# Orbis-Tertius/tiny-ram-halo2

Measured on AMD Instinct MI355X. Metric: Pallas MSM pairs/s @ 2^24 + Fp NTT elems/s @ 2^22; 1/2/4/8 MI355X, higher is better.
Workload: dtype u255 (255-bit modular integers as 9 x 29/30-bit limbs in i32 / i64 lanes)

## Files before the change

tiny-ram-halo2_amd/csrc/msm.hip:

```cpp
#include <stdlib.h>
#include <string.h>

#include "ctx.h"
#include "devmem.h"
#include "curve_q4.h"
#include "hostcombine.h"
#include "hosthelper.h"
#include "hostplan.h"

namespace trh {

namespace {

using hostplan::MAX_C; using hostplan::MAX_C_FIXED; using hostplan::MSM_TILE; using hostplan::SMALL_C; using hostplan::SMALL_MAX_N;
using hostplan::PART_TILE; using hostplan::BIN_THREADS; using hostplan::BIN_PER_MAX; using hostplan::BIN_CAP_MAX; using hostplan::RANGE_BLOCK;
using hostplan::HEAVY_PIECES; using hostplan::SP_LISTS; using hostplan::SP_CNT; using hostplan::SP_PAD; using hostplan::SP_PARTS; using hostplan::SP_MAX_CHUNK;
using hostplan::num_windows;
static_assert(sizeof(XYZZMem) == hostplan::XYZZ_BYTES && sizeof(XYZZzMem) == hostplan::RAW_POINT_BYTES, "point sizes of the plan's scratch layout");
constexpr u32 SIGN_BIT = 0x80000000u;

template <class SF>
__global__ void __launch_bounds__(256) msm_recode_kernel(const uint4* __restrict__ scalars, size_t n, int mont, int c, int W,
                                                         u32* __restrict__ digits, u32* __restrict__ bin_counts, int k2, u32 nbins, int use_lds, size_t sstride,
                                                         int one_row ,
                                                         const uint4* __restrict__ tails ,
                                                         unsigned char* __restrict__ tile_flags ,
                                                         u32 tile_log, u32 tiles) {
    const size_t z = blockIdx.z;
    const u32 rows = one_row ? 1u : (u32)W;
    scalars += z * sstride * 2; digits += z * (size_t)W * n; bin_counts += z * (size_t)rows * nbins;
    extern __shared__ u32 lhist[];
    const u32 total = rows * nbins;
    if (use_lds) {
        for (u32 k = threadIdx.x; k < total; k += blockDim.x) lhist[k] = 0;
        __syncthreads();
    }
    const u32 mask = (1u << c) - 1u, half = 1u << (c - 1);
    for (size_t i = (size_t)blockIdx.x * blockDim.x + threadIdx.x; i < n; i += (size_t)gridDim.x * blockDim.x) {
        const uint4* src = (tails && i == n - 1) ? tails + 2 * z : scalars + 2 * i;
        uint4 lo = src[0], hi = src[1];
        u32 w[8] = {lo.x, lo.y, lo.z, lo.w, hi.x, hi.y, hi.z, hi.w};
        if (mont) fe_store(fe_from_mont(fe_load<SF>(w)), w);
        u32 carry = 0;
        for (int j = 0; j < W; ++j) {
            u32 raw = (w[0] & mask) + carry;
#pragma unroll
            for (int k = 0; k < 7; ++k) w[k] = (w[k] >> c) | (w[k + 1] << (32 - c));
            w[7] >>= c;
            u32 bucket, sign = 0;
            if (raw > half) { bucket = (1u << c) - raw; carry = 1; sign = SIGN_BIT; }
            else { bucket = raw; carry = 0; }
            digits[(size_t)j * n + i] = bucket ? (bucket | sign) : 0u;
            if (tile_flags) {
                const unsigned long long nz = __ballot(bucket != 0);
                const size_t slot = (size_t)j * n + i;
                const u32 lane = threadIdx.x & 63u;
                if (bucket && ((nz & ((1ull << lane) - 1ull)) == 0ull || (slot & (((size_t)1 << tile_log) - 1)) < 64))
                    tile_flags[z * tiles + (slot >> tile_log)] = 1;
            }
            if (bucket) {
                const u32 bin = (bucket - 1u) >> k2, row = one_row ? 0u : (u32)j;
                if (use_lds) atomicAdd(&lhist[row * nbins + bin], 1u);
                else atomicAdd(&bin_counts[(size_t)row * nbins + bin], 1u);
            }
        }
    }
    if (use_lds) {
        __syncthreads();
        for (u32 k = threadIdx.x; k < total; k += blockDim.x) {
            const u32 v = lhist[k];
            if (v) atomicAdd(&bin_counts[k], v);
        }
    }
}

struct ZeroRanges { uint4* p[4]; u32 n16[4]; };
__global__ void __launch_bounds__(256) msm_zero_ranges_kernel(const ZeroRanges z) {
    const uint4 zero = make_uint4(0, 0, 0, 0);
#pragma unroll
    for (int k = 0; k < 4; ++k)
        for (u32 i = blockIdx.x * blockDim.x + threadIdx.x; i < z.n16[k]; i += gridDim.x * blockDim.x) z.p[k][i] = zero;
}

__global__ void __launch_bounds__(1024) msm_offsets_kernel(u32* __restrict__ counts, u32* __restrict__ starts, u32 nb1, u32* __restrict__ oversize, u32 bin_cap,
                                                           u32* __restrict__ totals ) {
    const size_t z = blockIdx.z;
    counts += z * (size_t)gridDim.x * nb1; starts += z * (size_t)gridDim.x * nb1;
    __shared__ u32 part[1024];
    const int j = blockIdx.x, t = threadIdx.x;
    u32* cnt = counts + (size_t)j * nb1;
    u32* st = starts + (size_t)j * nb1;
    const u32 per = (nb1 + 1023u) / 1024u;
    const u32 lo = t * per < nb1 ? t * per : nb1, hi = (lo + per < nb1) ? lo + per : nb1;
    u32 sum = 0, biggest = 0;
    for (u32 b = lo; b < hi; ++b) { const u32 v = cnt[b]; sum += v; biggest = v > biggest ? v : biggest; }
    if (oversize && biggest > bin_cap) atomicMax(oversize + z * gridDim.x + blockIdx.x, biggest);
    part[t] = sum;
    __syncthreads();
    for (int off = 1; off < 1024; off <<= 1) {
        u32 v = (t >= off) ? part[t - off] : 0;
        __syncthreads();
        part[t] += v;
        __syncthreads();
    }
    if (totals && t == 1023) totals[z * gridDim.x + blockIdx.x] = part[1023];
    u32 run = part[t] - sum;
    for (u32 b = lo; b < hi; ++b) {
        u32 cv = cnt[b];
        st[b] = run;
        cnt[b] = run;
        run += cv;
    }
}

constexpr int PART_THREADS = 1024;
__global__ void __launch_bounds__(PART_THREADS) msm_partition_kernel(const u32* __restrict__ digits, u32* __restrict__ bin_cursor,
                                                                     u32* __restrict__ parted, size_t n, int k2, u32 nbins, int idx_bits,
                                                                     const unsigned char* __restrict__ tile_flags ) {
    const size_t z = blockIdx.z;
    if (tile_flags && !tile_flags[z * gridDim.x + blockIdx.x]) return;
    digits += z * (size_t)gridDim.y * n; parted += z * (size_t)gridDim.y * n; bin_cursor += z * (size_t)gridDim.y * nbins;
    extern __shared__ u32 lds[];
    u32* stage = lds;
    u32* cnt = lds + PART_TILE;
    u32* lbase = cnt + nbins;
    u32* gbase = lbase + nbins;
    __shared__ u32 scan[PART_THREADS];
    const int j = blockIdx.y;
    const size_t t0 = (size_t)blockIdx.x * PART_TILE;
    const size_t t1 = t0 + PART_TILE < n ? t0 + PART_TILE : n;
    const u32* dg = digits + (size_t)j * n;
    for (u32 k = threadIdx.x; k < nbins; k += blockDim.x) cnt[k] = 0;
    __syncthreads();
    constexpr int PER = PART_TILE / PART_THREADS;
    u32 mine[PER];
#pragma unroll
    for (int q = 0; q < PER; ++q) {
        const size_t i = t0 + threadIdx.x + (size_t)q * PART_THREADS;
        mine[q] = i < t1 ? dg[i] : 0u;
    }
#pragma unroll
    for (int q = 0; q < PER; ++q) {
        const u32 b = mine[q] & ~SIGN_BIT;
        if (b) atomicAdd(&cnt[(b - 1u) >> k2], 1u);
    }
    __syncthreads();
    {
        const u32 per = (nbins + PART_THREADS - 1) / PART_THREADS;
        const u32 lo = threadIdx.x * per < nbins ? threadIdx.x * per : nbins, hi = lo + per < nbins ? lo + per : nbins;
        u32 sum = 0;
        for (u32 k = lo; k < hi; ++k) sum += cnt[k];
        scan[threadIdx.x] = sum;
        __syncthreads();
        for (int off = 1; off < PART_THREADS; off <<= 1) {
            const u32 v = ((int)threadIdx.x >= off) ? scan[threadIdx.x - off] : 0;
            __syncthreads();
            scan[threadIdx.x] += v;
            __syncthreads();
        }
        u32 run = scan[threadIdx.x] - sum;
        for (u32 k = lo; k < hi; ++k) {
            const u32 v = cnt[k];
            lbase[k] = run;
            gbase[k] = v ? atomicAdd(&bin_cursor[(size_t)j * nbins + k], v) : 0u;
            run += v;
        }
    }
    __syncthreads();
    for (u32 k = threadIdx.x; k < nbins; k += blockDim.x) cnt[k] = 0;
    __syncthreads();
    const u32 low_mask = (1u << k2) - 1u;
#pragma unroll
    for (int q = 0; q < PER; ++q) {
        const u32 e = mine[q];
        const u32 b = e & ~SIGN_BIT;
        if (b) {
            const u32 bm = b - 1u, bin = bm >> k2;
            const u32 r = atomicAdd(&cnt[bin], 1u);
            stage[lbase[bin] + r] = (u32)(t0 + threadIdx.x + (size_t)q * PART_THREADS) | ((bm & low_mask) << idx_bits) | (e & SIGN_BIT);
        }
    }
    __syncthreads();
    u32* out = parted + (size_t)j * n;
    const u32 wave = threadIdx.x >> 6, lane = threadIdx.x & 63u;
    for (u32 bin = wave; bin < nbins; bin += PART_THREADS / 64) {
        const u32 c = cnt[bin], lb = lbase[bin], gb = gbase[bin];
        for (u32 k = lane; k < c; k += 64) out[gb + k] = stage[lb + k];
    }
}

constexpr int BS_CHUNK = 8192;
constexpr int BS_THREADS = 512;

__device__ __forceinline__ u32 bin_of_position(const u32* __restrict__ bin_ends, u32 nbins, u32 pos) {
    u32 lo = 0, hi = nbins;
    while (lo < hi) {
        const u32 mid = (lo + hi) >> 1;
        if (bin_ends[mid] > pos) hi = mid; else lo = mid + 1;
    }
    return lo;
}

template <bool SCATTER>
__global__ void __launch_bounds__(BS_THREADS) msm_bucket_pass_kernel(const u32* __restrict__ parted, const u32* __restrict__ bin_starts,
                                                                     const u32* __restrict__ bin_ends, u32* __restrict__ bucket_cnt ,
                                                                     u32* __restrict__ sorted, size_t n, int k2, u32 nbins, int idx_bits, u32 nbk,
                                                                     const u32* __restrict__ oversize) {
    const size_t z = blockIdx.z;
    {
        const size_t Wz = gridDim.y;
        parted += z * Wz * n; sorted += z * Wz * n; bin_starts += z * Wz * nbins; bin_ends += z * Wz * nbins;
        bucket_cnt += z * Wz * (nbk + 1);
    }
    if (oversize && oversize[z * gridDim.y + blockIdx.y] == 0u) return;
    __shared__ u32 cnt[128], tbase[128], gbase[128];
    __shared__ u32 stage[SCATTER ? BS_CHUNK : 1];
    const int j = blockIdx.y;
    const u32* bs = bin_starts + (size_t)j * nbins;
    const u32* be = bin_ends + (size_t)j * nbins;
    const u32 total = be[nbins - 1];
    const u32 c0 = blockIdx.x * BS_CHUNK;
    if (c0 >= total) return;
    const u32 c1 = c0 + BS_CHUNK < total ? c0 + BS_CHUNK : total;
    const u32 nsub = 1u << k2, low_mask = nsub - 1u, idx_mask = (1u << idx_bits) - 1u;
    const u32* src = parted + (size_t)j * n;
    u32* dst = sorted + (size_t)j * n;
    u32* bc = bucket_cnt + (size_t)j * (nbk + 1);
    const u32 wave = threadIdx.x >> 6, lane = threadIdx.x & 63u;
    for (u32 bin = bin_of_position(be, nbins, c0); bin < nbins; ++bin) {
        const u32 lo = bs[bin] > c0 ? bs[bin] : c0;
        if (lo >= c1) break;
        const u32 hi = be[bin] < c1 ? be[bin] : c1;
        if (hi <= lo) continue;
        if (hi - lo <= 64u) {
            if (threadIdx.x < hi - lo) {
                const u32 e = src[lo + threadIdx.x];
                u32* cell = &bc[(bin << k2) + ((e >> idx_bits) & low_mask) + 1u];
                if (!SCATTER) atomicAdd(cell, 1u);
                else dst[atomicAdd(cell, 1u)] = (e & idx_mask) | (e & SIGN_BIT);
            }
            continue;
        }
        if (threadIdx.x < 128) cnt[threadIdx.x] = 0;
        __syncthreads();
        for (u32 i = lo + threadIdx.x; i < hi; i += blockDim.x) atomicAdd(&cnt[(src[i] >> idx_bits) & low_mask], 1u);
        __syncthreads();
        if (!SCATTER) {
            if (threadIdx.x < nsub && cnt[threadIdx.x]) atomicAdd(&bc[(bin << k2) + threadIdx.x + 1u], cnt[threadIdx.x]);
        } else {
            if (threadIdx.x == 0) {
                u32 r = 0;
                for (u32 k = 0; k < nsub; ++k) { tbase[k] = r; r += cnt[k]; }
            }
            if (threadIdx.x < nsub) {
                const u32 v = cnt[threadIdx.x];
                gbase[threadIdx.x] = v ? atomicAdd(&bc[(bin << k2) + threadIdx.x + 1u], v) : 0u;
            }
            __syncthreads();
            if (threadIdx.x < 128) cnt[threadIdx.x] = 0;
            __syncthreads();
            for (u32 i = lo + threadIdx.x; i < hi; i += blockDim.x) {
                const u32 e = src[i];
                const u32 sub = (e >> idx_bits) & low_mask;
                const u32 r = atomicAdd(&cnt[sub], 1u);
                stage[tbase[sub] + r] = (e & idx_mask) | (e & SIGN_BIT);
            }
            __syncthreads();
            for (u32 sub = wave; sub < nsub; sub += BS_THREADS / 64) {
                const u32 c = cnt[sub], sb = tbase[sub], gb = gbase[sub];
                for (u32 k = lane; k < c; k += 64) dst[gb + k] = stage[sb + k];
            }
        }
        __syncthreads();
    }
}

template <int PER>
__global__ void __launch_bounds__(BIN_THREADS) msm_bin_sort_kernel(const u32* __restrict__ parted, const u32* __restrict__ bin_starts, const u32* __restrict__ bin_ends,
                                                                   u32* __restrict__ sorted, u32* __restrict__ starts, u32* __restrict__ ends, size_t n, int k2, u32 nbins,
                                                                   int idx_bits, u32 nbk, const u32* __restrict__ oversize) {
    if (oversize[(size_t)blockIdx.z * gridDim.y + blockIdx.y] != 0u) return;
    extern __shared__ u32 bstage[];
    __shared__ u32 cnt[128], tbase[128], wave0_total;
    const size_t z = blockIdx.z, Wz = gridDim.y;
    const int j = blockIdx.y;
    const u32 bin = blockIdx.x;
    const size_t wrow = z * Wz + j;
    const u32 lo = bin_starts[wrow * nbins + bin], hi = bin_ends[wrow * nbins + bin];
    const u32 count = hi - lo;
    const u32 nsub = 1u << k2, low_mask = nsub - 1u, idx_mask = (1u << idx_bits) - 1u;
    const u32* src = parted + wrow * n + lo;
    u32* dst = sorted + wrow * n + lo;
    const u32 lane = threadIdx.x & 63u;
    if (threadIdx.x < 128) cnt[threadIdx.x] = 0;
    __syncthreads();
    u32 mine[PER];
#pragma unroll
    for (int q = 0; q < PER; ++q) {
        const u32 i = threadIdx.x + (u32)q * BIN_THREADS;
        mine[q] = (u32)q * BIN_THREADS < count ? src[i < count ? i : 0u] : 0u;
    }
#pragma unroll
    for (int q = 0; q < PER; ++q)
        if (threadIdx.x + (u32)q * BIN_THREADS < count) atomicAdd(&cnt[(mine[q] >> idx_bits) & low_mask], 1u);
    __syncthreads();
    u32 v = 0, x = 0;
    if (threadIdx.x < 128) {
        v = threadIdx.x < nsub ? cnt[threadIdx.x] : 0u;
        x = v;
#pragma unroll
        for (int off = 1; off < 64; off <<= 1) {
            const u32 y = __shfl_up(x, off, 64);
            if ((int)lane >= off) x += y;
        }
        if (threadIdx.x == 63) wave0_total = x;
    }
    __syncthreads();
    if (threadIdx.x < 128) {
        const u32 excl = x - v + (threadIdx.x >= 64 ? wave0_total : 0u);
        tbase[threadIdx.x] = excl;
        cnt[threadIdx.x] = 0;
        if (threadIdx.x < nsub) {
            const size_t b = wrow * (nbk + 1) + ((size_t)bin << k2) + threadIdx.x + 1u;
            starts[b] = lo + excl;
            ends[b] = lo + excl + v;
        }
        if (bin == 0 && threadIdx.x == 0) { starts[wrow * (nbk + 1)] = 0; ends[wrow * (nbk + 1)] = 0; }
    }
    __syncthreads();
#pragma unroll
    for (int q = 0; q < PER; ++q) {
        if (threadIdx.x + (u32)q * BIN_THREADS < count) {
            const u32 e = mine[q];
            const u32 sub = (e >> idx_bits) & low_mask;
            const u32 r = atomicAdd(&cnt[sub], 1u);
            bstage[tbase[sub] + r] = (e & idx_mask) | (e & SIGN_BIT);
        }
    }
    __syncthreads();
#pragma unroll
    for (int q = 0; q < PER; ++q) {
        const u32 i = threadIdx.x + (u32)q * BIN_THREADS;
        if (i < count) mine[q] = bstage[i];
    }
#pragma unroll
    for (int q = 0; q < PER; ++q) {
        const u32 i = threadIdx.x + (u32)q * BIN_THREADS;
        if (i < count) dst[i] = mine[q];
    }
}

__global__ void __launch_bounds__(RANGE_BLOCK) msm_bucket_block_sums_kernel(const u32* __restrict__ bucket_cnt, u32* __restrict__ block_sums, u32 nbk,
                                                                            const u32* __restrict__ oversize) {
    if (oversize && oversize[(size_t)blockIdx.z * gridDim.y + blockIdx.y] == 0u) return;
    __shared__ u32 part[RANGE_BLOCK / 64];
    const size_t z = blockIdx.z, Wz = gridDim.y;
    const u32 nb1 = nbk + 1, b = blockIdx.x * RANGE_BLOCK + threadIdx.x;
    u32 v = b < nb1 ? bucket_cnt[(z * Wz + blockIdx.y) * nb1 + b] : 0u;
#pragma unroll
    for (int off = 32; off > 0; off >>= 1) v += __shfl_down(v, off, 64);
    if ((threadIdx.x & 63) == 0) part[threadIdx.x >> 6] = v;
    __syncthreads();
    if (threadIdx.x == 0) {
        u32 t = 0;
        for (int k = 0; k < RANGE_BLOCK / 64; ++k) t += part[k];
        block_sums[(z * Wz + blockIdx.y) * gridDim.x + blockIdx.x] = t;
    }
}
__global__ void __launch_bounds__(RANGE_BLOCK) msm_bucket_ranges_kernel(u32* __restrict__ bucket_cnt, const u32* __restrict__ block_sums, u32* __restrict__ starts,
                                                                        u32* __restrict__ ends, u32 nbk, const u32* __restrict__ oversize) {
    if (oversize && oversize[(size_t)blockIdx.z * gridDim.y + blockIdx.y] == 0u) return;
    __shared__ u32 part[RANGE_BLOCK];
    __shared__ u32 before;
    const size_t z = blockIdx.z, Wz = gridDim.y;
    const int t = threadIdx.x;
    const u32 nb1 = nbk + 1, b = blockIdx.x * RANGE_BLOCK + t;
    const size_t row = (z * Wz + blockIdx.y) * nb1;
    const u32 c = b < nb1 ? bucket_cnt[row + b] : 0u;
    {
        u32 v = (u32)t < blockIdx.x ? block_sums[(z * Wz + blockIdx.y) * gridDim.x + t] : 0u;
        part[t] = v;
        __syncthreads();
        for (int s = RANGE_BLOCK / 2; s > 0; s >>= 1) {
            if (t < s) part[t] += part[t + s];
            __syncthreads();
        }
        if (t == 0) before = part[0];
        __syncthreads();
    }
    part[t] = c;
    __syncthreads();
    for (int off = 1; off < RANGE_BLOCK; off <<= 1) {
        const u32 v = (t >= off) ? part[t - off] : 0;
        __syncthreads();
        part[t] += v;
        __syncthreads();
    }
    if (b < nb1) {
        const u32 E = before + part[t], S = E - c;
        starts[row + b] = S; ends[row + b] = E; bucket_cnt[row + b] = S;
    }
}

template <class BF>
__device__ __forceinline__ void store_zrec(uint4* q, const Fy<BF>& x, const Fy<BF>& y) {
    q[0] = make_uint4((u32)x.l[0], (u32)x.l[1], (u32)x.l[2], (u32)x.l[3]); q[1] = make_uint4((u32)x.l[4], (u32)x.l[5], (u32)x.l[6], (u32)x.l[7]);
    q[2] = make_uint4((u32)y.l[0], (u32)y.l[1], (u32)y.l[2], (u32)y.l[3]); q[3] = make_uint4((u32)y.l[4], (u32)y.l[5], (u32)y.l[6], (u32)y.l[7]);
    q[4] = make_uint4((u32)-y.l[0], (u32)-y.l[1], (u32)-y.l[2], (u32)-y.l[3]); q[5] = make_uint4((u32)-y.l[4], (u32)-y.l[5], (u32)-y.l[6], (u32)-y.l[7]);
    q[6] = make_uint4((u32)x.l[8], (u32)y.l[8], (u32)-y.l[8], 0u);
    q[7] = make_uint4(0u, 0u, 0u, 0u);
}
template <class BF>
__global__ void __launch_bounds__(256) msm_convert_bases_kernel(const uint4* __restrict__ in, uint4* __restrict__ out, size_t n) {
    size_t i = (size_t)blockIdx.x * blockDim.x + threadIdx.x;
    if (i >= n) return;
    const uint4* p = in + i * 4;
    uint4 a = p[0], b = p[1], c = p[2], d = p[3];
    store_zrec(out + i * (ZREC / 16), fy_from_fe(fe_load<BF>(a.x, a.y, a.z, a.w, b.x, b.y, b.z, b.w)), fy_from_fe(fe_load<BF>(c.x, c.y, c.z, c.w, d.x, d.y, d.z, d.w)));
}

template <class BF>
__global__ void __launch_bounds__(256) msm_accumulate_seg_kernel(const uint4* __restrict__ bases_z, const u32* __restrict__ sorted,
                                                                 const u32* __restrict__ ends,
                                                                 XYZZzMem* __restrict__ first, XYZZzMem* __restrict__ last,
                                                                 XYZZzMem* __restrict__ direct, size_t n, u32 nbk, u32 nseg, u32 seg_len,
                                                                 const u32* __restrict__ lean_gate ) {
    const size_t z = blockIdx.z;
    if (lean_gate && lean_gate[z * gridDim.y + blockIdx.y] != 0u) return;
    {
        const size_t Wz = gridDim.y;
        sorted += z * Wz * n; ends += z * Wz * (nbk + 1);
        first += z * Wz * nseg; last += z * Wz * nseg; direct += z * Wz * (nbk + 1);
    }
    const u32 t = blockIdx.x * blockDim.x + threadIdx.x;
    const int j = blockIdx.y;
    if (t >= nseg) return;
    const u32 nb1 = nbk + 1;
    const u32* en = ends + (size_t)j * nb1;
    const u32 total = en[nbk];
    u32 pos = t * seg_len;
    if (pos >= total) return;
    const u32 stop = pos + seg_len < total ? pos + seg_len : total;
    u32 B;
    {
        u32 lo = 0, hi = nbk;
        while (lo < hi) {
            const u32 mid = (lo + hi) >> 1;
            if (en[mid] > pos) hi = mid; else lo = mid + 1;
        }
        B = lo;
    }
    u32 cur_end = en[B];
    const u32* lst = sorted + (size_t)j * n;
    XYZZzMem* my_first = first + (size_t)j * nseg + t;
    XYZZz<BF> acc = xyzzz_identity<BF>();
    bool is_first = true;
    bool fresh = true;
    struct Slot { u32 e; uint4 a, b, c, d, t; };
    auto issue = [&](Slot& sl, u32 entry) {
        sl.e = entry;
        const uint4* bp = bases_z + (size_t)(entry & ~SIGN_BIT) * (ZREC / 16);
        const uint4* yp = bp + 2 + ((entry >> 31) << 1);
        sl.a = bp[0]; sl.b = bp[1]; sl.c = yp[0]; sl.d = yp[1]; sl.t = bp[6];
    };
    auto unpack = [&](const Slot& sl, AffineZ<BF>& p) {
        p.x.l[0] = (i32)sl.a.x; p.x.l[1] = (i32)sl.a.y; p.x.l[2] = (i32)sl.a.z; p.x.l[3] = (i32)sl.a.w;
        p.x.l[4] = (i32)sl.b.x; p.x.l[5] = (i32)sl.b.y; p.x.l[6] = (i32)sl.b.z; p.x.l[7] = (i32)sl.b.w; p.x.l[8] = (i32)sl.t.x;
        p.y.l[0] = (i32)sl.c.x; p.y.l[1] = (i32)sl.c.y; p.y.l[2] = (i32)sl.c.z; p.y.l[3] = (i32)sl.c.w;
        p.y.l[4] = (i32)sl.d.x; p.y.l[5] = (i32)sl.d.y; p.y.l[6] = (i32)sl.d.z; p.y.l[7] = (i32)sl.d.w; p.y.l[8] = (i32)((sl.e >> 31) ? sl.t.z : sl.t.y);
    };
    const u32 last_pos = stop - 1;
    auto clamp = [&](u32 q) { return q < last_pos ? q : last_pos; };
    Slot s0, s1;
    issue(s0, lst[pos]);
    issue(s1, lst[clamp(pos + 1)]);
    u32 e_ahead = lst[clamp(pos + 2)];
    auto step = [&](Slot& sl) {
        if (pos == cur_end) {
            store_raw(is_first ? my_first : direct + (size_t)j * nb1 + B, acc);
            is_first = false;
            fresh = true;
            int walked = 0;
            do { ++B; cur_end = en[B]; } while (cur_end <= pos && ++walked < 4);
            if (cur_end <= pos) {
                u32 lo = B + 1, hi = nbk;
                while (lo < hi) {
                    const u32 mid = (lo + hi) >> 1;
                    if (en[mid] > pos) hi = mid; else lo = mid + 1;
                }
                B = lo;
// ... 1292 lines not shown
```

Baseline: 1.011 billion.

## Use wave-shuffle scan and batched per-wave bin copy in MSM partition kernel

The partition kernel's 1024-thread LDS prefix scan, which needed about 20 block barriers, becomes a 64-lane shuffle scan per wave plus a small cross-wave combine through LDS. The counter reset is folded into the base-computation loop, which removes one barrier. Global bases are stored as deltas. The final copy from LDS to global has each wave load metadata for up to 64 bins into lanes, broadcast it with readlane, and handle four bins per step, so loads are issued ahead of stores and short bins cost less. This adds code complexity, and readlane indexing must stay within the lanes that hold metadata.

```diff
diff --git a/tiny-ram-halo2_amd/csrc/msm.hip b/tiny-ram-halo2_amd/csrc/msm.hip
--- a/tiny-ram-halo2_amd/csrc/msm.hip
+++ b/tiny-ram-halo2_amd/csrc/msm.hip
@@ -124,12 +124,13 @@
     u32* stage = lds;
     u32* cnt = lds + PART_TILE;
     u32* lbase = cnt + nbins;
-    u32* gbase = lbase + nbins;
-    __shared__ u32 scan[PART_THREADS];
+    u32* gdelta = lbase + nbins;
+    __shared__ u32 wave_total[PART_THREADS / 64];
     const int j = blockIdx.y;
     const size_t t0 = (size_t)blockIdx.x * PART_TILE;
     const size_t t1 = t0 + PART_TILE < n ? t0 + PART_TILE : n;
     const u32* dg = digits + (size_t)j * n;
+    const u32 wave = threadIdx.x >> 6, lane = threadIdx.x & 63u;
     for (u32 k = threadIdx.x; k < nbins; k += blockDim.x) cnt[k] = 0;
     __syncthreads();
     constexpr int PER = PART_TILE / PART_THREADS;
@@ -145,29 +146,33 @@
         if (b) atomicAdd(&cnt[(b - 1u) >> k2], 1u);
     }
     __syncthreads();
+    u32 total;
     {
         const u32 per = (nbins + PART_THREADS - 1) / PART_THREADS;
         const u32 lo = threadIdx.x * per < nbins ? threadIdx.x * per : nbins, hi = lo + per < nbins ? lo + per : nbins;
         u32 sum = 0;
         for (u32 k = lo; k < hi; ++k) sum += cnt[k];
-        scan[threadIdx.x] = sum;
-        __syncthreads();
-        for (int off = 1; off < PART_THREADS; off <<= 1) {
-            const u32 v = ((int)threadIdx.x >= off) ? scan[threadIdx.x - off] : 0;
-            __syncthreads();
-            scan[threadIdx.x] += v;
-            __syncthreads();
-        }
-        u32 run = scan[threadIdx.x] - sum;
+        u32 x = sum;
+#pragma unroll
+        for (int off = 1; off < 64; off <<= 1) {
+            const u32 y = __shfl_up(x, off, 64);
+            if ((int)lane >= off) x += y;
+        }
+        if (lane == 63) wave_total[wave] = x;
+        __syncthreads();
+        u32 all = lane < PART_THREADS / 64 ? wave_total[lane] : 0u, before = lane < wave ? all : 0u;
+#pragma unroll
+        for (int off = PART_THREADS / 128; off > 0; off >>= 1) { all += __shfl_xor(all, off, 64); before += __shfl_xor(before, off, 64); }
+        total = __shfl(all, 0, 64);
+        u32 run = __shfl(before, 0, 64) + x - sum;
         for (u32 k = lo; k < hi; ++k) {
             const u32 v = cnt[k];
             lbase[k] = run;
-            gbase[k] = v ? atomicAdd(&bin_cursor[(size_t)j * nbins + k], v) : 0u;
+            gdelta[k] = (v ? atomicAdd(&bin_cursor[(size_t)j * nbins + k], v) : 0u) - run;
+            cnt[k] = 0;
             run += v;
         }
     }
-    __syncthreads();
-    for (u32 k = threadIdx.x; k < nbins; k += blockDim.x) cnt[k] = 0;
     __syncthreads();
     const u32 low_mask = (1u << k2) - 1u;
 #pragma unroll
@@ -182,10 +187,28 @@
     }
     __syncthreads();
     u32* out = parted + (size_t)j * n;
-    const u32 wave = threadIdx.x >> 6, lane = threadIdx.x & 63u;
-    for (u32 bin = wave; bin < nbins; bin += PART_THREADS / 64) {
-        const u32 c = cnt[bin], lb = lbase[bin], gb = gbase[bin];
-        for (u32 k = lane; k < c; k += 64) out[gb + k] = stage[lb + k];
+    constexpr u32 WAVES = PART_THREADS / 64;
+    const u32 wave_u = __builtin_amdgcn_readfirstlane(wave);
+    for (u32 base = wave_u; base < nbins; base += 64 * WAVES) {
+        const u32 own = base + lane * WAVES;
+        u32 c_v = 0, lb_v = 0, gd_v = 0;
+        if (own < nbins) { c_v = cnt[own]; lb_v = lbase[own]; gd_v = gdelta[own]; }
+        const u32 left = (nbins - base + WAVES - 1) / WAVES, nl = left < 64u ? left : 64u;
+        for (u32 l = 0; l < nl; l += 4) {
+            u32 c[4], lb[4], gd[4], val[4];
+#pragma unroll
+            for (int u = 0; u < 4; ++u) {
+                c[u] = __builtin_amdgcn_readlane(c_v, l + u); lb[u] = __builtin_amdgcn_readlane(lb_v, l + u); gd[u] = __builtin_amdgcn_readlane(gd_v, l + u);
+            }
+#pragma unroll
+            for (int u = 0; u < 4; ++u) val[u] = lane < c[u] ? stage[lb[u] + lane] : 0u;
+#pragma unroll
+            for (int u = 0; u < 4; ++u)
+                if (lane < c[u]) out[gd[u] + lb[u] + lane] = val[u];
+#pragma unroll
+            for (int u = 0; u < 4; ++u)
+                for (u32 k = lane + 64; k < c[u]; k += 64) out[gd[u] + lb[u] + k] = stage[lb[u] + k];
+        }
     }
 }
 
```

Result: no change. 1.007 billion (median of 2 runs) (-0.4%).
